# panshengyi/MemVul

Hardware: AMD Instinct MI355X
Metric: issue-reports/sec at seq_len=256 (BERT-base issue encoder + 124-anchor memory match) (higher is better)
Workload: dtype fp16 + fp8 (MV_F16X8: fp16 MFMA sweep + one OCP-e4m3 MFMA correction sweep per GEMM, fp32 accumulate); 1 GPU; BASELINE.json configs[1]: 1xMI355X-per-rank, bert-base-uncased geometry (12 layers), seq_len=256, batch=256, 124-anchor CWE memory, compute dtype MV_F16X8; seeded random-init weights, synthetic token ids resident in HBM; compute=precise, global_batch=256, seq_len=256, anchors=124, parallelism=dp1 (corpus shards, one all-gather of (score,label) stats), stats_transport=none (one rank)

## Files before the change

### memvul_amd/binding.py

```python
from __future__ import annotations

import ctypes as C
import os
import warnings
from typing import Dict, Iterable, Optional, Tuple

import numpy as np

_HERE = os.path.dirname(os.path.abspath(__file__))
LIB_PATH = os.path.join(_HERE, "lib", "libmemvul_hip.so")
LIB_PATH_DEV = os.path.join(_HERE, "lib", "libmemvul_hip_dev.so")
DEV_SWITCHES = ("MEMVUL_GEMM_TILE", "MEMVUL_SHORT_VLO", "MEMVUL_RASTER", "MEMVUL_GN_MAX", "MEMVUL_NUM_CU")

MV_F32, MV_F16, MV_BF16, MV_I32, MV_I64 = 0, 1, 2, 3, 4
MV_F16X8 = 6
COMPUTE_DTYPES = {"f16": MV_F16, "fast": MV_F16, "f16x8": MV_F16X8, "precise": MV_F16X8, "safe": MV_F16X8, "guarded": MV_F16X8,
                  "f32": MV_F32, "reference": MV_F32}
MV_FORM_DEFAULT, MV_FORM_SAFE, MV_FORM_GUARDED = 0, 1, 2
FORMS = {"default": MV_FORM_DEFAULT, "safe": MV_FORM_SAFE, "guarded": MV_FORM_GUARDED}
GUARDED_WARN_SHARE = 0.25
DEFAULT_COMPUTE = "precise"


def default_compute() -> str:
    return os.environ.get("MEMVUL_COMPUTE", DEFAULT_COMPUTE)


def compute_dtype_of(name_or_code) -> int:
    if name_or_code is None:
        name_or_code = default_compute()
    if isinstance(name_or_code, str):
        if name_or_code.lower() not in COMPUTE_DTYPES:
            raise ValueError(f"unknown compute dtype {name_or_code!r}: expected one of {sorted(COMPUTE_DTYPES)}")
        return COMPUTE_DTYPES[name_or_code.lower()]
    if int(name_or_code) not in (MV_F16, MV_F16X8, MV_F32):
        raise ValueError(f"unknown compute dtype code {name_or_code!r}: MV_F16 = {MV_F16}, MV_F16X8 = {MV_F16X8} or MV_F32 = {MV_F32}")
    return int(name_or_code)


def on_sink_policy() -> str:
    v = os.environ.get("MEMVUL_ON_SINK", "warn")
    if v not in ("warn", "safe"):
        raise ValueError(f"MEMVUL_ON_SINK={v!r}: expected 'warn' or 'safe'")
    return v

# ... 607 lines not shown
```

### memvul_amd/csrc/engine.hip

```cpp
#include <hip/hip_runtime.h>
#include <dlfcn.h>
#include <rccl/rccl.h>
#include <unistd.h>

#include <algorithm>
#include <charconv>
#include <chrono>
#include <cmath>
#include <cstdio>
#include <cstdlib>
#include <cstring>
#include <map>
#include <string>
#include <vector>

#include "../../include/memvul_hip.h"
#include "common.h"
#include "gemm.h"
#include "gemm_pp.h"
#include "attention.h"
#include "attention_v2.h"
#include "misc_kernels.h"
#include "match_topk.h"
#include "ref_f32.h"
// ... 158 lines not shown
  int rr = 0;
  Plan plan;
  struct {
    std::vector<int32_t> ids, lens, idx;
    std::vector<float> logits, probs, best, embed;
    std::vector<uint32_t> over;
  } stage, stage2;
  Plan plan2;
  std::vector<uint8_t> last_forms;
  int64_t guard_seqs = 0, guard_rescored = 0;
  float* anchors = nullptr;
  int n_anchors = 0;
  unsigned long long* attn_conc = nullptr;
  unsigned long long* x8_sat = nullptr;

  int32_t *c_ids = nullptr, *c_lens = nullptr;
  std::vector<int32_t> c_lens_host;
  std::vector<void*> pinned;
  int64_t c_n = 0;
  int c_S = 0;
  float* c_best = nullptr;
  int32_t* c_idx = nullptr;
  float* c_psame = nullptr;
  int64_t c_psame_rows = 0;
  int c_G = 0;
  uint32_t* c_over = nullptr;
  std::vector<int16_t> c_pend_w;
  std::vector<uint8_t> c_pend_keep;
  std::vector<uint8_t> c_forms;
  bool c_pending = false;

  bool cls_prune = true;
  int pp_gn_max = 4;
  int pp_raster = 0;
  bool short_vlo = true;
  bool cls_aside = true;
  int cls_min_len = 128;
  int qkv_aside_mask = 0;

  int form = MV_FORM_DEFAULT;

  uint32_t prof_mask = 0xffffffffu;
  bool prof = false;
  std::vector<ProfRec> recs;
  std::vector<hipEvent_t> free_events;

  int gemm_tile = 0;
  int num_cu = 256;

  int dbg_B = 0, dbg_Sp = 0;

  void* rccl_lib = nullptr;
  ncclComm_t comm = nullptr;
  int comm_rank = 0, comm_world = 1;
  decltype(&ncclGetUniqueId) p_ncclGetUniqueId = nullptr;
  decltype(&ncclCommInitRank) p_ncclCommInitRank = nullptr;
  decltype(&ncclAllGather) p_ncclAllGather = nullptr;
  decltype(&ncclCommDestroy) p_ncclCommDestroy = nullptr;
  decltype(&ncclGetErrorString) p_ncclGetErrorString = nullptr;
  decltype(&ncclGetVersion) p_ncclGetVersion = nullptr;
  decltype(&ncclCommCount) p_ncclCommCount = nullptr;
  decltype(&ncclCommUserRank) p_ncclCommUserRank = nullptr;
  void *comm_send = nullptr, *comm_recv = nullptr;
  int64_t comm_send_cap = 0, comm_recv_cap = 0;
};

// ... 87 lines not shown
  hipError_t e = hipGetLastError();
  if (e != hipSuccess) return fail(h, MV_ERR_HIP, std::string("launch ") + what + ": " + hipGetErrorString(e));
  return MV_OK;
}

int choose_gn(int tn, int gn_max) {
  int g = 1;
  for (int d = 1; d <= gn_max && d <= tn; ++d)
    if (tn % d == 0) g = d;
  return g;
}

template <int EPI>
int launch_gemm128(mv_handle* h, hipStream_t stream, int cls, GemmArgs a) {
  if (a.M % 128 || a.N % 128 || a.K % 64) return fail(h, MV_ERR_INVALID, "gemm128: M,N % 128, K % 64 required");
  a.GN = choose_gn(a.N / 128, 8);
  const int grid = (a.M / 128) * (a.N / 128);
  ProfScope ps(h, stream, cls);
  hipLaunchKernelGGL((gemm128_kernel<EPI>), dim3(grid), dim3(256), G128_LDS_BYTES, stream, a);
  return launch_check(h, "gemm128");
}

constexpr int RING64_LDS = 4 * (64 + 64) * 64 * 2;
template <int EPI>
int launch_ring64(mv_handle* h, hipStream_t stream, int cls, GemmArgs a) {
  if (a.M % 64 || a.N % 64 || a.K % 64) return fail(h, MV_ERR_INVALID, "gemm_ring: shape not a multiple of the 64 x 64 x 64 tile");
  a.GN = choose_gn(a.N / 64, 8);
  const int grid = (a.M / 64) * (a.N / 64);
  ProfScope ps(h, stream, cls);
  hipLaunchKernelGGL((gemm_ring_kernel<EPI, 1, 1, 2, 2, 64, 4, 2>), dim3(grid), dim3(256), RING64_LDS, stream, a);
  return launch_check(h, "gemm_ring");
}

template <int PPEPI>
int launch_pp(mv_handle* h, hipStream_t stream, int cls, GemmArgs a) {
  constexpr int RAW = PPEPI != PP_RESLN3;
  if (a.M % 256 || a.N % 256 || a.K % 128 || a.K < 256 || a.N > MV_INTER)
    return fail(h, MV_ERR_INVALID, "gemm_pp: M,N % 256, K % 128, K >= 256, N <= 3072 required");
  if (!a.bias || !a.lnstats) return fail(h, MV_ERR_STATE, "internal: gemm_pp without bias / row statistics");
  if (a.A8 && (a.x8_terms == 1 || a.x8_terms == 3) && a.K % 256)
    return fail(h, MV_ERR_INVALID, "gemm_pp: a weight-side-only fp8 correction sweep needs K % 256 == 0");
  a.GN = choose_gn(a.N / 256, h->pp_gn_max);
  const int tiles = (a.M / 256) * (a.N / 256);
  const int grid = tiles < h->num_cu ? tiles : h->num_cu;
  a.raster_mode = (h->pp_raster == 1 && a.N / 256 > a.GN && ((a.M / 256) * a.GN) % grid == 0) ? 1 : 0;
  const int lds = RAW ? PP_LDS_BYTES_RAW : PP_LDS_BYTES;
  ProfScope ps(h, stream, cls);
  if (a.A8) {
    if (!a.W8 || (PPEPI != PP_QK && !a.out8)) return fail(h, MV_ERR_STATE, "internal: MV_F16X8 GEMM without its fp8 planes");
    hipLaunchKernelGGL((gemm_pp_kernel<PPEPI, RAW, 1>), dim3(grid), dim3(512), lds, stream, a);
  } else {
    hipLaunchKernelGGL((gemm_pp_kernel<PPEPI, RAW, 0>), dim3(grid), dim3(512), lds, stream, a);
  }
  return launch_check(h, "gemm_pp");
}

bool pp_selected(const mv_handle* h, int64_t M) {
  if (M % 256) return false;
  if (h->gemm_tile == 128) return false;
  return h->gemm_tile == 512 || h->precise || (M / 256) * (MV_HIDDEN / 256) >= 256;
}

template <int EPI>
int launch_small(mv_handle* h, hipStream_t stream, int cls, const GemmArgs& a) {
  if (h->gemm_tile == 0 && a.M <= 512 && a.M % 64 == 0 && a.N % 64 == 0) return launch_ring64<EPI>(h, stream, cls, a);
  return launch_gemm128<EPI>(h, stream, cls, a);
}

int pool_head(mv_handle* h, Work& wk, const float* x, size_t row_stride, int B, float* u_out) {
  const unsigned gx = (unsigned)((B + 31) / 32);
  hipLaunchKernelGGL(dense768_kernel<0>, dim3(gx, MV_HIDDEN / 32), dim3(512), 0, wk.stream, x, row_stride, B, h->WpT, h->bp,
                     MV_HIDDEN, h->P == MV_HIDDEN ? u_out : wk.pooled);
  if (int rc = launch_check(h, "pooler")) return rc;
  if (h->P == MV_HIDDEN) return MV_OK;
  hipLaunchKernelGGL(dense768_kernel<1>, dim3(gx, MV_PROJ / 32), dim3(512), 0, wk.stream, wk.pooled, (size_t)MV_HIDDEN, B, h->WhT,
                     h->bh, MV_PROJ, u_out);
  return launch_check(h, "header");
}

// ... 114 lines not shown
  }
  return MV_OK;
}

int encode_dev(mv_handle* h, Work& wk, const int32_t* d_ids, const int32_t* d_lens, int min_len, int B, int S_in, int n_layers, float* u_out,
               const PassForm& pf = PassForm(), bool full = false, int pitch = 0) {
  if (pitch <= 0) pitch = S_in;
  if (h->f32) return encode_f32_dev(h, wk, d_ids, d_lens, B, S_in, n_layers, u_out, pitch);
  const mv_config& c = h->cfg;
  const int Sp = padded_len(S_in);
  const int64_t M = (int64_t)B * Sp, Mpad = round_up(M, 256);
  if (S_in > c.max_pos) return fail(h, MV_ERR_INVALID, "sequence longer than max_pos");
  if (Mpad > h->cap_tokens) return fail(h, MV_ERR_CAPACITY, "B*S exceeds mv_config.max_tokens");
  if (n_layers < 0 || n_layers > c.layers) n_layers = c.layers;
  h->dbg_B = B;
  h->dbg_Sp = Sp;
  const bool big = pp_selected(h, Mpad);
  const bool x8 = h->precise;
  const bool prune = !full && h->cls_prune && u_out && n_layers == c.layers && n_layers > 0;
  const bool one_seq_tiles = Sp == 256 || Sp == 512;
  const bool whole_pass = (Sp == 192 || Sp == 384) && min_len >= h->cls_min_len;
  const bool safe = x8 && pf.safe;
  const bool cls_as = big && x8 && !safe && h->cls_aside && (one_seq_tiles || whole_pass);
  const int qkv_mask = safe ? 7 : h->qkv_aside_mask;
  const bool two_plane = two_plane_pass(h, x8, safe, Sp);
  if (cls_as && one_seq_tiles) {
    const int ntile = (int)(Mpad / 256);
    hipLaunchKernelGGL(cls_tile_flags_kernel, dim3((unsigned)((ntile + 255) / 256)), dim3(256), 0, wk.stream, d_lens, B, Sp, h->cls_min_len, ntile,
                       wk.tile_both);
    if (int rc = launch_check(h, "cls_tile_flags")) return rc;
  }
  const bool special = big && x8;
  auto row_term = [&](const half_t* A, const half_t* W, int N, int K) -> int {
    ProfScope ps(h, wk.stream, KC_CLS_ROW_TERM);
    GemmArgs t{};
    t.M = (int)round_up(2 * B, 64); t.Mreal = 2 * B; t.S = 64; t.A = A; t.W = W; t.N = N; t.K = K; t.outf = wk.cls_corr;
    t.GN = choose_gn(N / 64, 8);
    hipLaunchKernelGGL((gemm_ring_kernel<EPI_F32, 1, 1, 2, 2, 64, 4, 2>), dim3((unsigned)((t.M / 64) * (N / 64))), dim3(256), RING64_LDS, wk.stream, t);
    return launch_check(h, "row term gemm_ring");
  };
  const unsigned ln_grid = (unsigned)((M + 3) / 4);
  {
    ProfScope ps(h, wk.stream, KC_EMBED_LN);
    if (big)
      hipLaunchKernelGGL(embed_ln_kernel<true>, dim3(ln_grid), dim3(256), 0, wk.stream, d_ids, pitch, S_in, Sp, (int)M, c.vocab_size,
                         h->wemb, h->pemb, h->temb, h->embg, h->embb, c.ln_eps, wk.xres, wk.x16, wk.lnstats,
                         x8 ? (half_t*)nullptr : wk.xlo, x8 ? wk.x8 : (uint8_t*)nullptr, h->x8_sat, special ? d_lens : (const int32_t*)nullptr,
                         special ? wk.st_lo : (half_t*)nullptr);
    else
      hipLaunchKernelGGL(embed_ln_kernel<false>, dim3(ln_grid), dim3(256), 0, wk.stream, d_ids, pitch, S_in, Sp, (int)M, c.vocab_size,
                         h->wemb, h->pemb, h->temb, h->embg, h->embb, c.ln_eps, wk.xres, wk.x16, (float*)nullptr,
                         (half_t*)nullptr, (uint8_t*)nullptr, (unsigned long long*)nullptr);
    if (int rc = launch_check(h, "embed_ln")) return rc;
  }
  const float *pend_g = h->embg, *pend_b = h->embb;
  auto run_ln = [&](float* x32, half_t* x16, int rows, const float* g, const float* b) -> int {
    ProfScope ps(h, wk.stream, KC_LN);
    hipLaunchKernelGGL(ln_kernel<true>, dim3((unsigned)((rows + 3) / 4)), dim3(256), 0, wk.stream, x32, x16, rows, g, b, c.ln_eps,
                       (float*)nullptr);
    return launch_check(h, "layernorm");
  };
  auto final_ln = [&](const float* g, const float* b) -> int {
    const size_t n4 = (size_t)M * MV_HIDDEN / 4;
    hipLaunchKernelGGL(hilo_to_f32_kernel, dim3((unsigned)((n4 + 255) / 256)), dim3(256), 0, wk.stream, wk.x16, wk.xlo, n4, wk.xres,
                       special ? (const half_t*)wk.st_lo : (const half_t*)nullptr, Sp, (const uint8_t*)wk.x8);
    if (int rc = launch_check(h, "hilo_to_f32")) return rc;
    return run_ln(wk.xres, wk.x16, (int)M, g, b);
  };
  if (big && n_layers == 0) { if (int rc = final_ln(h->embg, h->embb)) return rc; }
// ... 615 lines not shown
      g_create_error = std::string(name) + "=\"" + e + "\": expected an integer in " + std::to_string(lo) + " .. " + std::to_string(hi);
      return false;
    }
    *out = (int)v;
    return true;
  };
  auto env_flag = [&](const char* name, bool* out) -> bool {
    int v = *out ? 1 : 0;
    if (!env_int(name, 0, 1, &v)) return false;
    *out = v != 0;
    return true;
  };
  {
    int ns = h->n_streams;
    if (!env_int("MEMVUL_STREAMS", 1, 2, &ns)) return MV_ERR_INVALID;
    h->n_streams = h->n_alloc = ns;
  }
  for (int wi = 0; wi < h->n_alloc; ++wi) {
    e = hipStreamCreateWithFlags(&h->work[wi].stream, hipStreamNonBlocking);
    if (e != hipSuccess) {
      g_create_error = std::string("hipStreamCreate: ") + hipGetErrorString(e);
      return MV_ERR_HIP;
    }
  }
  hipFuncSetAttribute((const void*)gemm_ring_kernel<EPI_F32, 1, 1, 2, 2, 64, 4, 2>, hipFuncAttributeMaxDynamicSharedMemorySize, RING64_LDS);
  hipFuncSetAttribute((const void*)gemm_ring_kernel<EPI_QKV, 1, 1, 2, 2, 64, 4, 2>, hipFuncAttributeMaxDynamicSharedMemorySize, RING64_LDS);
  hipFuncSetAttribute((const void*)gemm_ring_kernel<EPI_GELU, 1, 1, 2, 2, 64, 4, 2>, hipFuncAttributeMaxDynamicSharedMemorySize, RING64_LDS);
  hipFuncSetAttribute((const void*)gemm_ring_kernel<EPI_RES, 1, 1, 2, 2, 64, 4, 2>, hipFuncAttributeMaxDynamicSharedMemorySize, RING64_LDS);
  hipFuncSetAttribute((const void*)gemm_pp_kernel<PP_QK, 1, 0>, hipFuncAttributeMaxDynamicSharedMemorySize, PP_LDS_BYTES_RAW);
  hipFuncSetAttribute((const void*)gemm_pp_kernel<PP_GELU, 1, 0>, hipFuncAttributeMaxDynamicSharedMemorySize, PP_LDS_BYTES_RAW);
  hipFuncSetAttribute((const void*)gemm_pp_kernel<PP_RESLN3, 0, 0>, hipFuncAttributeMaxDynamicSharedMemorySize, PP_LDS_BYTES);
  hipFuncSetAttribute((const void*)gemm_pp_kernel<PP_QK, 1, 1>, hipFuncAttributeMaxDynamicSharedMemorySize, PP_LDS_BYTES_RAW);
  hipFuncSetAttribute((const void*)gemm_pp_kernel<PP_GELU, 1, 1>, hipFuncAttributeMaxDynamicSharedMemorySize, PP_LDS_BYTES_RAW);
  hipFuncSetAttribute((const void*)gemm_pp_kernel<PP_RESLN3, 0, 1>, hipFuncAttributeMaxDynamicSharedMemorySize, PP_LDS_BYTES);
#define MV_ATT_ATTR(NKB, NCH)                                                                                                     \
  hipFuncSetAttribute((const void*)attention_v2_kernel<NKB, NCH, 0>, hipFuncAttributeMaxDynamicSharedMemorySize, ATT2_LDS_BYTES(NKB)); \
  hipFuncSetAttribute((const void*)attention_v2_kernel<NKB, NCH, 1>, hipFuncAttributeMaxDynamicSharedMemorySize, ATT2_LDS_BYTES(NKB))
  MV_ATT_ATTR(1, 1); MV_ATT_ATTR(2, 1); MV_ATT_ATTR(3, 1); MV_ATT_ATTR(4, 1); MV_ATT_ATTR(2, 3); MV_ATT_ATTR(2, 4);
#undef MV_ATT_ATTR
  hipFuncSetAttribute((const void*)attention_v2_kernel<1, 1, 1, 1>, hipFuncAttributeMaxDynamicSharedMemorySize, ATT2_LDS_BYTES_VLO(1));
  hipFuncSetAttribute((const void*)attention_v2_kernel<2, 1, 1, 1>, hipFuncAttributeMaxDynamicSharedMemorySize, ATT2_LDS_BYTES_VLO(2));
  hipFuncSetAttribute((const void*)attention_v2_kernel<1, 3, 1, 1>, hipFuncAttributeMaxDynamicSharedMemorySize, ATT2_LDS_BYTES_VLO(1));
  hipFuncSetAttribute((const void*)attention_v2_kernel<2, 2, 1, 1>, hipFuncAttributeMaxDynamicSharedMemorySize, ATT2_LDS_BYTES_VLO(2));
  hipFuncSetAttribute((const void*)attention_v2_kernel<2, 3, 1, 1>, hipFuncAttributeMaxDynamicSharedMemorySize, ATT2_LDS_BYTES_VLO(2));
  hipFuncSetAttribute((const void*)attention_v2_kernel<2, 4, 1, 1>, hipFuncAttributeMaxDynamicSharedMemorySize, ATT2_LDS_BYTES_VLO(2));
  (void)hipGetLastError();
  if (!env_flag("MEMVUL_CLS_PRUNE", &h->cls_prune)) return MV_ERR_INVALID;
  if (const char* e = getenv("MEMVUL_QKV_ASIDE")) {
    h->qkv_aside_mask = 0;
    if (strcmp(e, "none")) {
      for (const char* c = e; *c; ++c) {
        const int bit = (*c == 'q' || *c == 'Q') ? 1 : (*c == 'k' || *c == 'K') ? 2 : (*c == 'v' || *c == 'V') ? 4 : 0;
        if (!bit) {
          g_create_error = std::string("MEMVUL_QKV_ASIDE=\"") + e + "\": expected a subset of \"qkv\", \"\" or \"none\"";
          return MV_ERR_INVALID;
        }
        h->qkv_aside_mask |= bit;
      }
    }
  }
  if (!env_flag("MEMVUL_CLS_ASIDE", &h->cls_aside)) return MV_ERR_INVALID;
  if (!env_int("MEMVUL_CLS_ASIDE_MIN_LEN", 1, 512, &h->cls_min_len)) return MV_ERR_INVALID;
  if (const char* e = getenv("MEMVUL_FORM")) {
    if (!strcmp(e, "safe")) h->form = MV_FORM_SAFE;
    else if (!strcmp(e, "default")) h->form = MV_FORM_DEFAULT;
    else if (!strcmp(e, "guarded")) h->form = MV_FORM_GUARDED;
    else {
      g_create_error = std::string("MEMVUL_FORM=\"") + e + "\": expected \"default\", \"safe\" or \"guarded\"";
      return MV_ERR_INVALID;
    }
  }
  {
    int ncu = 0;
    if (hipDeviceGetAttribute(&ncu, hipDeviceAttributeMultiprocessorCount, device) == hipSuccess && ncu > 0) h->num_cu = ncu;
  }
#ifdef MEMVUL_DEV_SWITCHES
  {
    int gt = h->gemm_tile;
    if (!env_int("MEMVUL_GEMM_TILE", 0, 512, &gt)) return MV_ERR_INVALID;
    if (gt != 0 && gt != 128 && gt != 512) { g_create_error = "MEMVUL_GEMM_TILE: expected 0, 128 or 512"; return MV_ERR_INVALID; }
    h->gemm_tile = gt;
    if (!env_flag("MEMVUL_SHORT_VLO", &h->short_vlo)) return MV_ERR_INVALID;
    if (!env_int("MEMVUL_GN_MAX", 1, 12, &h->pp_gn_max)) return MV_ERR_INVALID;
    if (!env_int("MEMVUL_RASTER", 0, 1, &h->pp_raster)) return MV_ERR_INVALID;
    if (!env_int("MEMVUL_NUM_CU", 1, h->num_cu, &h->num_cu)) return MV_ERR_INVALID;
  }
#endif

  h->cap_tokens = round_up(cfg->max_tokens, 256) + 256;
  const int64_t T = h->cap_tokens;
  int rc = MV_OK;
  auto A = [&](int r) { if (rc == MV_OK) rc = r; };
  const int64_t BG = (int64_t)cfg->max_batch * cfg->max_anchors;
  const int64_t Bp = round_up(cfg->max_batch, 256);
  for (int wi = 0; wi < h->n_alloc; ++wi) {
    Work& wk = h->work[wi];
    A(dev_alloc(h, wk.stream, &wk.d_ids, T));
    A(dev_alloc(h, wk.stream, &wk.d_lens, (int64_t)cfg->max_batch + 16));
    A(dev_alloc(h, wk.stream, &wk.seq_over, (int64_t)cfg->max_batch));
    A(dev_alloc(h, wk.stream, &wk.d_idx, (int64_t)cfg->max_batch));
    A(dev_alloc(h, wk.stream, &wk.xres, T * MV_HIDDEN));
    A(dev_alloc(h, wk.stream, &wk.x16, T * MV_HIDDEN));
    A(dev_alloc(h, wk.stream, &wk.q, T * MV_HIDDEN));
    A(dev_alloc(h, wk.stream, &wk.k, T * MV_HIDDEN));
    A(dev_alloc(h, wk.stream, &wk.vt, T * MV_HIDDEN));
    A(dev_alloc(h, wk.stream, &wk.ctx, T * MV_HIDDEN));
    A(dev_alloc(h, wk.stream, &wk.h16, T * MV_INTER));
    A(dev_alloc(h, wk.stream, &wk.lnstats, T * 6));
    A(dev_alloc(h, wk.stream, &wk.lnpart, T * 6));
    A(dev_alloc(h, wk.stream, &wk.c32, Bp * MV_HIDDEN));
    A(dev_alloc(h, wk.stream, &wk.cq, Bp * MV_HIDDEN));
    A(dev_alloc(h, wk.stream, &wk.c16, Bp * MV_HIDDEN));
    A(dev_alloc(h, wk.stream, &wk.cctx, Bp * MV_HIDDEN));
    A(dev_alloc(h, wk.stream, &wk.ch16, Bp * MV_INTER));
    A(dev_alloc(h, wk.stream, &wk.u, (int64_t)cfg->max_batch * h->P));
    A(dev_alloc(h, wk.stream, &wk.pooled, (int64_t)cfg->max_batch * MV_HIDDEN));
    A(dev_alloc(h, wk.stream, &wk.u_in, (int64_t)cfg->max_batch * h->P));
// ... 781 lines not shown

int mv_debug_read(mv_handle* h, int buffer, void* dst, int64_t bytes) try {
  if (!h || !dst || bytes <= 0) return MV_ERR_INVALID;
  Work& wk = h->work[0];
  const int64_t T = (int64_t)h->dbg_B * h->dbg_Sp;
  const void* src = nullptr;
  int64_t avail = 0;
  if (h->f32 && buffer >= 1 && buffer <= 9)
    return fail(h, MV_ERR_INVALID, "mv_debug_read: buffers 1 - 9 are the fp16 planes of MV_F16 / MV_F16X8; an MV_F32 handle has buffer 0 (hidden fp32) and 10 (embedding)");
  switch (buffer) {
    case 0: src = wk.xres; avail = T * MV_HIDDEN * 4; break;
    case 1: src = wk.x16; avail = T * MV_HIDDEN * 2; break;
    case 2: src = wk.q; avail = T * MV_HIDDEN * 2; break;
    case 3: src = wk.k; avail = T * MV_HIDDEN * 2; break;
    case 4: src = wk.vt; avail = T * MV_HIDDEN * 2; break;
    case 5: src = wk.ctx; avail = T * MV_HIDDEN * 2; break;
    case 6: src = wk.h16; avail = T * MV_INTER * 2; break;
    case 7: src = wk.q_lo; avail = T * MV_HIDDEN * 2; break;
    case 8: src = wk.k_lo; avail = T * MV_HIDDEN * 2; break;
    case 9: src = wk.vt_lo; avail = T * MV_HIDDEN * 2; break;
    case 10: src = wk.u; avail = (int64_t)h->dbg_B * h->P * 4; break;
    default: return fail(h, MV_ERR_INVALID, "mv_debug_read: unknown buffer");
  }
  if (!src) return fail(h, MV_ERR_STATE, "mv_debug_read: this buffer does not exist in this compute dtype");
  if (bytes > avail) return fail(h, MV_ERR_INVALID, "mv_debug_read: more bytes requested than the buffer holds");
  HIPCHK(h, hipMemcpyAsync(dst, src, (size_t)bytes, hipMemcpyDeviceToHost, wk.stream));
  HIPCHK(h, hipStreamSynchronize(wk.stream));
  return MV_OK;
} catch (...) { return on_exception(h); }

int mv_test_gemm(mv_handle* h, int variant, int M, int N, int K, const uint16_t* A, const uint16_t* W, const float* bias,
                 float* C, int iters, float* ms) try {
  if (!h || !A || !W || M <= 0 || N <= 0 || K <= 0) return fail(h, MV_ERR_INVALID, "mv_test_gemm: bad argument");
  if (variant != 0 && variant != 19) return fail(h, MV_ERR_INVALID, "mv_test_gemm: variant 0 (128^2 tile) or 19 (64^2 ring)");
  if (variant == 0 && (M % 128 || N % 128 || K % 64)) return fail(h, MV_ERR_INVALID, "mv_test_gemm: M,N % 128 and K % 64 required");
  HIPCHK(h, hipSetDevice(h->device));
  const hipStream_t s0 = h->work[0].stream;
  half_t *dA = nullptr, *dW = nullptr;
  float *dB = nullptr, *dC = nullptr;
  int rc;
  if ((rc = dev_alloc(h, s0, &dA, (int64_t)M * K, false))) return rc;
  if ((rc = dev_alloc(h, s0, &dW, (int64_t)N * K, false))) return rc;
  if ((rc = dev_alloc(h, s0, &dB, N))) return rc;
  if ((rc = dev_alloc(h, s0, &dC, (int64_t)M * N))) return rc;
  HIPCHK(h, hipMemcpyAsync(dA, A, (size_t)M * K * 2, hipMemcpyHostToDevice, s0));
  HIPCHK(h, hipMemcpyAsync(dW, W, (size_t)N * K * 2, hipMemcpyHostToDevice, s0));
  if (bias) HIPCHK(h, hipMemcpyAsync(dB, bias, (size_t)N * 4, hipMemcpyHostToDevice, s0));
  GemmArgs g{};
  g.A = dA; g.W = dW; g.bias = dB; g.M = M; g.Mreal = M; g.N = N; g.K = K; g.outf = dC; g.S = 64;
  if (iters < 1) iters = 1;
  hipEvent_t e0, e1;
  hipEventCreate(&e0);
  hipEventCreate(&e1);
  auto run = [&]() -> int { return variant == 0 ? launch_gemm128<EPI_F32>(h, s0, KC_TEST_GEMM, g) : launch_ring64<EPI_F32>(h, s0, KC_TEST_GEMM, g); };
  rc = run();
  if (rc == MV_OK) {
    hipEventRecord(e0, s0);
    for (int i = 0; i < iters && rc == MV_OK; ++i) rc = run();
    hipEventRecord(e1, s0);
  }
  hipError_t se = hipStreamSynchronize(s0);
  float t = 0.f;
  hipEventElapsedTime(&t, e0, e1);
  hipEventDestroy(e0);
  hipEventDestroy(e1);
  if (ms) *ms = t / (float)iters;
  if (rc == MV_OK && se != hipSuccess) rc = fail(h, MV_ERR_HIP, std::string("test gemm: ") + hipGetErrorString(se));
  if (rc == MV_OK && C) {
    se = hipMemcpy(C, dC, (size_t)M * N * 4, hipMemcpyDeviceToHost);
    if (se != hipSuccess) rc = fail(h, MV_ERR_HIP, std::string("test gemm copy: ") + hipGetErrorString(se));
  }
  dev_free(h, dA); dev_free(h, dW); dev_free(h, dB); dev_free(h, dC);
  return rc;
} catch (...) { return on_exception(h); }

int mv_test_gemm_f32(mv_handle* h, int act, int M, int N, int K, const float* A, const float* W, const float* bias, const float* res, float* C, int iters,
                     float* ms) try {
  if (!h || !A || !W || M <= 0 || N <= 0 || K <= 0) return fail(h, MV_ERR_INVALID, "mv_test_gemm_f32: bad argument");
  if (act < RF_ACT_NONE || act > RF_ACT_RES || (act == RF_ACT_RES && !res)) return fail(h, MV_ERR_INVALID, "mv_test_gemm_f32: act 0 (bias), 1 (GELU) or 2 (+ res, res required)");
  if (M % 128 || N % 128 || K % 32) return fail(h, MV_ERR_INVALID, "mv_test_gemm_f32: M,N % 128 and K % 32 required");
  HIPCHK(h, hipSetDevice(h->device));
  const hipStream_t s0 = h->work[0].stream;
  float *dA = nullptr, *dW = nullptr, *dB = nullptr, *dR = nullptr, *dC = nullptr;
  int rc;
  if ((rc = dev_alloc(h, s0, &dA, (int64_t)M * K, false))) return rc;
  if ((rc = dev_alloc(h, s0, &dW, (int64_t)N * K, false))) return rc;
  if ((rc = dev_alloc(h, s0, &dB, N))) return rc;
// ... 202 lines not shown
```

### memvul_amd/csrc/gemm.h

```cpp
#pragma once
#include "common.h"

enum { EPI_F32 = 0, EPI_QKV = 1, EPI_GELU = 2, EPI_RES = 3 };

struct GemmArgs {
  const half_t* A;
  const half_t* W;
  const float* bias;
  int M;
  int Mreal;
  int N, K;
  int GN;
  float* outf;
  half_t* out16;
  half_t* out16b;
  float* xres;
  half_t* q;
  half_t* k;
  half_t* vt;
  int S;
  int col0;
  const float* lnstats;
  const float* lng;
  const float* lnb;
  float* lnpart;
  float ln_eps;
  const uint8_t* A8;
  const uint8_t* W8;
  uint8_t* out8;
  int x8_scale;
  int x8_terms;
  int x8_aside_mask;
  half_t* vt_lo;
  half_t *q_lo, *k_lo;
  unsigned long long* x8_sat;
  int raster_mode;
  int out8_hi_only;
  const int* tile_both;
  const float* cls_corr;
  half_t* sp_lo_out;
  half_t* vlo_sp;
};

__device__ __forceinline__ void raster(int t, int tm_count, int tn_count, int GN, int& tile_m, int& tile_n) {
  const int per_group = tm_count * GN;
  const int g = t / per_group;
  const int r = t - g * per_group;
  tile_m = r / GN;
  tile_n = g * GN + (r - tile_m * GN);
}

template <int EPI>
__device__ __forceinline__ void epilogue_frag(const GemmArgs& a, const floatx16& acc, int mb, int nb, int lane) {
  const int hi = lane >> 5;
  const int n = nb + (lane & 31);
  if constexpr (EPI == EPI_F32) {
#pragma unroll
    for (int r = 0; r < 16; ++r) a.outf[(size_t)(mb + mfma32_row(r, hi)) * a.N + n] = acc[r];
  } else if constexpr (EPI == EPI_GELU) {
#pragma unroll
    for (int r = 0; r < 16; ++r) a.out16[(size_t)(mb + mfma32_row(r, hi)) * a.N + n] = (half_t)gelu_erf(acc[r]);
  } else if constexpr (EPI == EPI_RES) {
    const int lane_off = 4 * hi * MV_HIDDEN + (lane & 31);
#pragma unroll
    for (int r = 0; r < 16; ++r) {
      float* rowbase = a.xres + (size_t)(mb + (r & 3) + 8 * (r >> 2)) * MV_HIDDEN + nb;
      rowbase[lane_off] = acc[r];
    }
  } else {
    const int which = (nb + a.col0) / MV_HIDDEN;
    const int hn = nb + a.col0 - which * MV_HIDDEN;
    const int head = hn >> 6;
// ... 202 lines not shown
#pragma unroll
        for (int j = 0; j < FR_N; ++j)
          acc[i][j] = __builtin_amdgcn_mfma_f32_32x32x16_f16(fa[i], fb[j], acc[i][j], 0, 0, 0);
    }
  };

  const int nk = K / BK;
#pragma unroll
  for (int s = 0; s < STAGES - 1; ++s)
    if (s < nk) stage(s, s);
  int slot = 0, fill = STAGES - 1;
  for (int kt = 0; kt < nk; ++kt) {
    const int newer = nk - 1 - kt;
    if (STAGES >= 5 && newer >= 3) wait_vmcnt<(STAGES >= 5 ? 3 : 0) * G>();
    else if (STAGES >= 4 && newer >= 2) wait_vmcnt<(STAGES >= 4 ? 2 : 0) * G>();
    else if (STAGES >= 3 && newer >= 1) wait_vmcnt<(STAGES >= 3 ? 1 : 0) * G>();
    else wait_vmcnt<0>();
    asm volatile("s_waitcnt lgkmcnt(0)" ::: "memory");
    __builtin_amdgcn_s_barrier();
    asm volatile("" ::: "memory");
    if (kt + STAGES - 1 < nk) stage(fill, kt + STAGES - 1);
    compute(slot);
    asm volatile("" ::: "memory");
    slot = (slot + 1 == STAGES) ? 0 : slot + 1;
    fill = (fill + 1 == STAGES) ? 0 : fill + 1;
  }

#pragma unroll
  for (int i = 0; i < FR_M; ++i)
#pragma unroll
    for (int j = 0; j < FR_N; ++j)
      epilogue_frag<EPI>(a, acc[i][j], m0 + (wm * FR_M + i) * 32, n0 + (wn * FR_N + j) * 32, lane);
}
```

### memvul_amd/csrc/gemm_pp.h

```cpp
#pragma once
#include "common.h"
#include <type_traits>
#include "gemm.h"

enum { PP_QK = 1, PP_GELU = 3, PP_RESLN3 = 8 };
constexpr int PP_F = 4;

#define PP_LDS_A 0
#define PP_LDS_B 65536
#define PP_LDS_BIAS 131072
#define PP_LDS_SCR (PP_LDS_BIAS + MV_INTER * 4)
#define PP_LDS_BYTES (PP_LDS_SCR + 8 * 2048)
#define PP_LDS_BIAS_T PP_LDS_BIAS
#define PP_LDS_STATS (PP_LDS_BIAS + 2048)
#define PP_LDS_SCR_RAW (PP_LDS_STATS + 2 * 6144)
#define PP_LDS_RSTD (PP_LDS_SCR_RAW + 8 * 2048)
#define PP_LDS_BYTES_RAW (PP_LDS_RSTD + 2048)

__device__ __forceinline__ uint32_t pack_h2(float a, float b) {
  const half2_t h = {(half_t)a, (half_t)b};
  return __builtin_bit_cast(uint32_t, h);
}

__device__ __forceinline__ void pin_f32x4(float& a, float& b, float& c, float& d) {
#if defined(__HIP_DEVICE_COMPILE__)
  asm("" : "+v"(a), "+v"(b), "+v"(c), "+v"(d));
#endif
}

__device__ __forceinline__ uint32_t f2u(float x) { return __float_as_uint(x); }
__device__ __forceinline__ float u2f(uint32_t x) { return __uint_as_float(x); }
typedef uint32_t u32x2 __attribute__((ext_vector_type(2)));
typedef uint32_t u32x4 __attribute__((ext_vector_type(4)));
typedef int intx4 __attribute__((ext_vector_type(4)));
typedef int intx8 __attribute__((ext_vector_type(8)));

__device__ __forceinline__ void scr_f16x2(uint32_t w0, uint32_t w1, uint32_t w2, uint32_t w3, const u32x2 (&da)[4],
                                          const u32x2 (&db)[4], uint32_t r, u32x4 (&o)[4]) {
#if defined(__HIP_DEVICE_COMPILE__)
  asm volatile(
      "ds_write_b64 %4, %8\n\tds_write_b64 %5, %9\n\tds_write_b64 %6, %10\n\tds_write_b64 %7, %11\n\t"
      "ds_read_b128 %0, %16\n\tds_read_b128 %1, %16 offset:1024\n\t"
      "ds_write_b64 %4, %12\n\tds_write_b64 %5, %13\n\tds_write_b64 %6, %14\n\tds_write_b64 %7, %15\n\t"
      "ds_read_b128 %2, %16\n\tds_read_b128 %3, %16 offset:1024\n\ts_waitcnt lgkmcnt(0)"
      : "=&v"(o[0]), "=&v"(o[1]), "=&v"(o[2]), "=&v"(o[3])
// ... 52 lines not shown
}
__device__ __forceinline__ void scr_f16_rev2(uint32_t wc, const u32x4& a0, const u32x4& a1, const u32x4& b0, const u32x4& b1, uint32_t r0,
                                             uint32_t r1, uint32_t r2, uint32_t r3, u32x2 (&oa)[4], u32x2 (&ob)[4]) {
#if defined(__HIP_DEVICE_COMPILE__)
  asm volatile(
      "ds_write_b128 %8, %9\n\tds_write_b128 %8, %10 offset:1024\n\t"
      "ds_read_b64 %0, %13\n\tds_read_b64 %1, %14\n\tds_read_b64 %2, %15\n\tds_read_b64 %3, %16\n\t"
      "ds_write_b128 %8, %11\n\tds_write_b128 %8, %12 offset:1024\n\t"
      "ds_read_b64 %4, %13\n\tds_read_b64 %5, %14\n\tds_read_b64 %6, %15\n\tds_read_b64 %7, %16\n\ts_waitcnt lgkmcnt(0)"
      : "=&v"(oa[0]), "=&v"(oa[1]), "=&v"(oa[2]), "=&v"(oa[3]), "=&v"(ob[0]), "=&v"(ob[1]), "=&v"(ob[2]), "=&v"(ob[3])
      : "v"(wc), "v"(a0), "v"(a1), "v"(b0), "v"(b1), "v"(r0), "v"(r1), "v"(r2), "v"(r3)
      : "memory");
  __builtin_amdgcn_sched_barrier(0);
#endif
}


__device__ __forceinline__ void lds_read_bgb1(uint32_t addr, float4& bi, float4& ga, float4& be) {
#if defined(__HIP_DEVICE_COMPILE__)
  asm volatile("ds_read_b128 %0, %3\n\tds_read_b128 %1, %3 offset:3072\n\tds_read_b128 %2, %3 offset:6144\n\ts_waitcnt lgkmcnt(0)"
               : "=&v"(bi), "=&v"(ga), "=&v"(be)
               : "v"(addr)
               : "memory");
  __builtin_amdgcn_sched_barrier(0);
#endif
}

__device__ __forceinline__ int sload_i32(const int* p) {
  int v = 0;
#if defined(__HIP_DEVICE_COMPILE__)
  asm volatile("s_load_dword %0, %1, 0x0\n\ts_waitcnt lgkmcnt(0)" : "=s"(v) : "s"(p) : "memory");
#endif
  return v;
}

__device__ __forceinline__ void raster_pp(const GemmArgs& a, int L, int G, int tm_count, int tn_count, int& tile_m, int& tile_n) {
  if (a.raster_mode == 1) {
    const int ngroups = tn_count / a.GN;
    const int w = L / G, r = L - w * G;
    const int b = w / ngroups, g = w - b * ngroups;
    const int p = b * G + r;
    tile_m = p / a.GN;
    tile_n = g * a.GN + (p - tile_m * a.GN);
  } else {
    raster(L, tm_count, tn_count, a.GN, tile_m, tile_n);
  }
}

template <int EPI, int RAW = 0, int X8 = 0>
__global__ __launch_bounds__(512, 2) void gemm_pp_kernel(GemmArgs a) {
  static_assert(EPI == PP_QK || EPI == PP_GELU || EPI == PP_RESLN3, "kernel kinds of the encoder layer");
  static_assert(RAW == (EPI != PP_RESLN3), "PP_QK / PP_GELU consume the raw stream (virtual LayerNorm), PP_RESLN3 produces it");
  constexpr bool IS_RES = (EPI == PP_RESLN3);
  static_assert(X8 == 0 || X8 == 1, "X8 = 1: MV_F16X8 (the fp8 correction sweep)");
  constexpr int WAITN = 2 * PP_F;
  constexpr int LDS_SCR = RAW ? PP_LDS_SCR_RAW : PP_LDS_SCR;
  extern __shared__ __attribute__((aligned(16))) char smem[];
  const int tid = threadIdx.x;
  const int lane = tid & 63;
  const int hi = lane >> 5, l31 = lane & 31;
  const int wave = __builtin_amdgcn_readfirstlane(tid >> 6);
  const int wr = wave >> 2, wc = wave & 3;
  const int K = a.K, nk0 = K >> 6;
  constexpr int nseg = X8 ? 2 : 1;
  auto short_tile = [&](int tm) -> bool { return a.tile_both && sload_i32(a.tile_both + tm) != 0; };
  auto both_terms = [&](int tm, int tn) -> bool {
// ... 236 lines not shown
    if constexpr (X8) {
#if defined(__HIP_DEVICE_COMPILE__)
      constexpr int P = s & 3, a0 = (P >= 2) ? 4 : 0, bq = (P == 1 || P == 2) ? 2 : 0;
      asm volatile("" : "+v"(acc[a0][bq]), "+v"(acc[a0 + 1][bq]), "+v"(acc[a0 + 2][bq]), "+v"(acc[a0 + 3][bq]), "+v"(acc[a0][bq + 1]),
                   "+v"(acc[a0 + 1][bq + 1]), "+v"(acc[a0 + 2][bq + 1]), "+v"(acc[a0 + 3][bq + 1]));
#endif
    }
    asm volatile("s_waitcnt vmcnt(%0)" ::"n"(WAITN) : "memory");
    __builtin_amdgcn_sched_barrier(0);
    __builtin_amdgcn_s_barrier();
    __builtin_amdgcn_sched_barrier(0);
  };

  auto issue_stats = [&](int itn, int tm, int tn) {
    if (itn * G + bslot < ntiles && wave < 4) {
#pragma unroll
      for (int pc = 0; pc < 2; ++pc) {
        const int piece = 2 * wave + pc;
        if (piece < 6) {
          const char* src = (const char*)a.lnstats + (size_t)tm * 6144 + piece * 1024 + lane * 16;
          glds16((const half_t*)src, smem + PP_LDS_STATS + (itn & 1) * 6144 + piece * 1024);
        } else if (piece == 6) {
          const char* src = (const char*)a.bias + (size_t)tn * 1024 + lane * 16;
          glds16((const half_t*)src, smem + PP_LDS_BIAS_T + (itn & 1) * 1024);
        }
      }
    }
  };
  if constexpr (RAW) {
    int tm = 0, tn = 0;
    if (bslot < ntiles) raster_pp(a, bslot, G, tm_count, tn_count, tm, tn);
    issue_stats(0, tm, tn);
  }

  issue_psi(std::integral_constant<int, 0>{});
  issue_psi(std::integral_constant<int, 1>{});
  issue_psi(std::integral_constant<int, 2>{});
  issue_psi(std::integral_constant<int, 3>{});
  issue_psi(std::integral_constant<int, 4>{});
  issue_psi(std::integral_constant<int, 5>{});
  issue_psi(std::integral_constant<int, 6>{});
  asm volatile("s_waitcnt vmcnt(%0) lgkmcnt(0)" ::"n"(WAITN) : "memory");
  __builtin_amdgcn_sched_barrier(0);
  __builtin_amdgcn_s_barrier();
  __builtin_amdgcn_sched_barrier(0);

  auto run_tiles = [&](auto grpc) {
  for (int it = 0;; ++it) {
    const int L = it * G + bslot;
    if (L >= ntiles) break;
    int tile_m, tile_n;
    raster_pp(a, L, G, tm_count, tn_count, tile_m, tile_n);
    int next_m = 0, next_n = 0;
    const bool has_next = L + G < ntiles;
    if (has_next) raster_pp(a, L + G, G, tm_count, tn_count, next_m, next_n);
    const int mw = (tile_m << 8) + wr * 128;
    const int nw = (tile_n << 8) + wc * 64;
    bool tile_short = false;
    if constexpr (X8) tile_short = short_tile(tile_m);
    const bool tile_both_terms = X8 && (a.x8_terms == 1 ? tile_short : both_terms(tile_m, tile_n));

    {
      const uint32_t baddr = (uint32_t)(PP_LDS_BIAS + (nw + 4 * q4) * 4);
      const uint32_t scr = (uint32_t)(LDS_SCR + wave * 2048);
      const uint32_t sf = (uint32_t)((m16 >> 2) & 3);
      const uint32_t scr_c = scr + (lane >> 2) * 64 + ((((uint32_t)lane & 3) ^ (((uint32_t)lane >> 4) & 3)) << 4);
// ... 79 lines not shown
          }
      }
    }

    if constexpr (decltype(grpc)::value == 0) read_set(std::integral_constant<int, 0>{});
    auto two_ktiles = [&](auto f8c, bool last) {
      interval(std::integral_constant<int, 0>{}, grpc, f8c);
      interval(std::integral_constant<int, 1>{}, grpc, f8c);
      interval(std::integral_constant<int, 2>{}, grpc, f8c);
      interval(std::integral_constant<int, 3>{}, grpc, f8c);
      interval(std::integral_constant<int, 4>{}, grpc, f8c);
      interval(std::integral_constant<int, 5>{}, grpc, f8c);
      interval(std::integral_constant<int, 6>{}, grpc, f8c);
      interval(std::integral_constant<int, 7>{}, grpc, f8c, last);
    };
    for (int kt = 0; kt < nk0; kt += 2) {
      if constexpr (RAW) {
        if (kt == 2) {
          issue_stats(it + 1, next_m, next_n);
          if (wave >= 4) {
            const int row = (wave - 4) * 64 + lane;
            const uint32_t saddr = (uint32_t)(PP_LDS_STATS + (it & 1) * 6144 + row * 24);
            float2 p0, p1, p2;
            asm volatile("ds_read_b64 %0, %3\n\tds_read_b64 %1, %3 offset:8\n\tds_read_b64 %2, %3 offset:16\n\ts_waitcnt lgkmcnt(0)"
                         : "=&v"(p0), "=&v"(p1), "=&v"(p2)
                         : "v"(saddr)
                         : "memory");
            const float rs = ln_from_partials(p0, p1, p2, a.ln_eps).y;
            const uint32_t waddr = (uint32_t)(PP_LDS_RSTD + (it & 1) * 1024 + row * 4);
            asm volatile("ds_write_b32 %0, %1" ::"v"(waddr), "v"(rs) : "memory");
          }
        }
      }
      two_ktiles(std::false_type{}, !X8 && kt + 2 >= nk0);
    }
    if constexpr (X8) {
      const int nk = nk0 + (tile_both_terms ? nk0 : nk0 >> 1);
      for (int kt = nk0; kt < nk; kt += 2) two_ktiles(std::true_type{}, kt + 2 >= nk);
    }

    {
      const uint32_t scr = (uint32_t)(LDS_SCR + wave * 2048);
      const uint32_t sf = (uint32_t)((m16 >> 2) & 3);
      const uint32_t scr_c = scr + (lane >> 2) * 64 + ((((uint32_t)lane & 3) ^ (((uint32_t)lane >> 4) & 3)) << 4);
      const int crow = lane >> 2, cchunk = lane & 3;
      int cls_b[2] = {-1, -1};
      if constexpr (X8) {
        if (a.cls_corr || a.sp_lo_out || a.vlo_sp) {
#pragma unroll
          for (int j = 0; j < 2; ++j) {
            const int row = mw + 64 * j, b = row / a.S;
            if (row < a.Mreal && b * a.S == row) cls_b[j] = b;
          }
        }
        if (a.cls_corr && !tile_both_terms) {
#pragma unroll
          for (int j = 0; j < 2; ++j) {
            if (cls_b[j] >= 0 && m16 < 2) {
              const float* cp = a.cls_corr + (size_t)(2 * cls_b[j] + m16) * a.N + nw + 4 * q4;
              floatx4 c[4];
#pragma unroll
              for (int cb = 0; cb < 4; ++cb) c[cb] = *(const floatx4*)(cp + 16 * cb);
#if defined(__HIP_DEVICE_COMPILE__)
              asm volatile("" : "+v"(c[0]), "+v"(c[1]), "+v"(c[2]), "+v"(c[3]));
#endif
#pragma unroll
              for (int cb = 0; cb < 4; ++cb) {
                acc[4 * j][cb][0] = __builtin_fmaf(c[cb][0], 1.0f / 2048.0f, acc[4 * j][cb][0]);
                acc[4 * j][cb][1] = __builtin_fmaf(c[cb][1], 1.0f / 2048.0f, acc[4 * j][cb][1]);
                acc[4 * j][cb][2] = __builtin_fmaf(c[cb][2], 1.0f / 2048.0f, acc[4 * j][cb][2]);
                acc[4 * j][cb][3] = __builtin_fmaf(c[cb][3], 1.0f / 2048.0f, acc[4 * j][cb][3]);
              }
            }
          }
        }
      }
      if constexpr (IS_RES) {
#pragma unroll
        for (int tb = 0; tb < 8; ++tb) {
          float s1 = 0.f, s2 = 0.f;
#pragma unroll
          for (int cb = 0; cb < 4; ++cb)
#pragma unroll
            for (int e = 0; e < 4; ++e) {
              const float v = acc[tb][cb][e];
              s1 += v;
              s2 = __builtin_fmaf(v, v, s2);
            }
// ... 265 lines not shown
```

Before: 14500 issue-reports/s.

## Add dedicated row-term MFMA kernel and stage CLS correction via LDS prefetch

Replaces the 64x64 ring GEMM used for the small CLS row-term correction with a dedicated register-pipelined 32x32 MFMA kernel that streams A and W fragments directly from global memory without LDS. In the fp8-corrected pp GEMM, the per-tile CLS correction rows are prefetched into LDS mid-K-loop by two waves and read back in the epilogue, instead of each wave loading them from global memory at the end. Both paths are on by default (form 3) and aim to cut the row-term launch cost and the epilogue global-load latency. The trade-off is a larger LDS footprint for the RESLN3 variant and extra inline asm that must index correctly.

```diff
diff --git a/memvul_amd/binding.py b/memvul_amd/binding.py
--- a/memvul_amd/binding.py
+++ b/memvul_amd/binding.py
@@ -10,7 +10,7 @@
 _HERE = os.path.dirname(os.path.abspath(__file__))
 LIB_PATH = os.path.join(_HERE, "lib", "libmemvul_hip.so")
 LIB_PATH_DEV = os.path.join(_HERE, "lib", "libmemvul_hip_dev.so")
-DEV_SWITCHES = ("MEMVUL_GEMM_TILE", "MEMVUL_SHORT_VLO", "MEMVUL_RASTER", "MEMVUL_GN_MAX", "MEMVUL_NUM_CU")
+DEV_SWITCHES = ("MEMVUL_GEMM_TILE", "MEMVUL_SHORT_VLO", "MEMVUL_RASTER", "MEMVUL_GN_MAX", "MEMVUL_NUM_CU", "MEMVUL_ROW_TERM")
 
 MV_F32, MV_F16, MV_BF16, MV_I32, MV_I64 = 0, 1, 2, 3, 4
 MV_F16X8 = 6
diff --git a/memvul_amd/csrc/engine.hip b/memvul_amd/csrc/engine.hip
--- a/memvul_amd/csrc/engine.hip
+++ b/memvul_amd/csrc/engine.hip
@@ -214,6 +214,7 @@
 
   bool cls_prune = true;
   int pp_gn_max = 4;
+  int row_term_form = 3;
   int pp_raster = 0;
   bool short_vlo = true;
   bool cls_aside = true;
@@ -367,6 +368,16 @@
   return launch_check(h, "gemm_ring");
 }
 
+template <int WM, int WN, int D>
+int launch_row_term_t(mv_handle* h, hipStream_t stream, int cls, const GemmArgs& a) {
+  if (a.Mreal <= 0 || a.N % (32 * WN) || a.K % 64) return fail(h, MV_ERR_INVALID, "row_term: N % 32 WN, K % 64 required");
+  const int grid = ((a.Mreal + 32 * WM - 1) / (32 * WM)) * (a.N / (32 * WN));
+  ProfScope ps(h, stream, cls);
+  hipLaunchKernelGGL((row_term_kernel<WM, WN, D>), dim3((unsigned)grid), dim3(64 * WM * WN), 0, stream, a);
+  return launch_check(h, "row_term");
+}
+int launch_row_term(mv_handle* h, hipStream_t stream, int cls, const GemmArgs& a) { return launch_row_term_t<1, 2, 6>(h, stream, cls, a); }
+
 template <int PPEPI>
 int launch_pp(mv_handle* h, hipStream_t stream, int cls, GemmArgs a) {
   constexpr int RAW = PPEPI != PP_RESLN3;
@@ -379,7 +390,8 @@
   const int tiles = (a.M / 256) * (a.N / 256);
   const int grid = tiles < h->num_cu ? tiles : h->num_cu;
   a.raster_mode = (h->pp_raster == 1 && a.N / 256 > a.GN && ((a.M / 256) * a.GN) % grid == 0) ? 1 : 0;
-  const int lds = RAW ? PP_LDS_BYTES_RAW : PP_LDS_BYTES;
+  a.cls_lds = (h->row_term_form & 2) && a.A8 && a.cls_corr && a.S % 256 == 0 && a.K >= 384;
+  const int lds = RAW ? PP_LDS_BYTES_RAW : (a.A8 ? PP_LDS_BYTES_CORR : PP_LDS_BYTES);
   ProfScope ps(h, stream, cls);
   if (a.A8) {
     if (!a.W8 || (PPEPI != PP_QK && !a.out8)) return fail(h, MV_ERR_STATE, "internal: MV_F16X8 GEMM without its fp8 planes");
@@ -560,9 +572,10 @@
   }
   const bool special = big && x8;
   auto row_term = [&](const half_t* A, const half_t* W, int N, int K) -> int {
-    ProfScope ps(h, wk.stream, KC_CLS_ROW_TERM);
     GemmArgs t{};
     t.M = (int)round_up(2 * B, 64); t.Mreal = 2 * B; t.S = 64; t.A = A; t.W = W; t.N = N; t.K = K; t.outf = wk.cls_corr;
+    if (h->row_term_form & 1) return launch_row_term(h, wk.stream, KC_CLS_ROW_TERM, t);
+    ProfScope ps(h, wk.stream, KC_CLS_ROW_TERM);
     t.GN = choose_gn(N / 64, 8);
     hipLaunchKernelGGL((gemm_ring_kernel<EPI_F32, 1, 1, 2, 2, 64, 4, 2>), dim3((unsigned)((t.M / 64) * (N / 64))), dim3(256), RING64_LDS, wk.stream, t);
     return launch_check(h, "row term gemm_ring");
@@ -1244,7 +1257,7 @@
   hipFuncSetAttribute((const void*)gemm_pp_kernel<PP_RESLN3, 0, 0>, hipFuncAttributeMaxDynamicSharedMemorySize, PP_LDS_BYTES);
   hipFuncSetAttribute((const void*)gemm_pp_kernel<PP_QK, 1, 1>, hipFuncAttributeMaxDynamicSharedMemorySize, PP_LDS_BYTES_RAW);
   hipFuncSetAttribute((const void*)gemm_pp_kernel<PP_GELU, 1, 1>, hipFuncAttributeMaxDynamicSharedMemorySize, PP_LDS_BYTES_RAW);
-  hipFuncSetAttribute((const void*)gemm_pp_kernel<PP_RESLN3, 0, 1>, hipFuncAttributeMaxDynamicSharedMemorySize, PP_LDS_BYTES);
+  hipFuncSetAttribute((const void*)gemm_pp_kernel<PP_RESLN3, 0, 1>, hipFuncAttributeMaxDynamicSharedMemorySize, PP_LDS_BYTES_CORR);
 #define MV_ATT_ATTR(NKB, NCH)                                                                                                     \
   hipFuncSetAttribute((const void*)attention_v2_kernel<NKB, NCH, 0>, hipFuncAttributeMaxDynamicSharedMemorySize, ATT2_LDS_BYTES(NKB)); \
   hipFuncSetAttribute((const void*)attention_v2_kernel<NKB, NCH, 1>, hipFuncAttributeMaxDynamicSharedMemorySize, ATT2_LDS_BYTES(NKB))
@@ -1295,6 +1308,7 @@
     if (!env_flag("MEMVUL_SHORT_VLO", &h->short_vlo)) return MV_ERR_INVALID;
     if (!env_int("MEMVUL_GN_MAX", 1, 12, &h->pp_gn_max)) return MV_ERR_INVALID;
     if (!env_int("MEMVUL_RASTER", 0, 1, &h->pp_raster)) return MV_ERR_INVALID;
+    if (!env_int("MEMVUL_ROW_TERM", 0, 3, &h->row_term_form)) return MV_ERR_INVALID;
     if (!env_int("MEMVUL_NUM_CU", 1, h->num_cu, &h->num_cu)) return MV_ERR_INVALID;
   }
 #endif
@@ -2142,7 +2156,7 @@
 int mv_test_gemm(mv_handle* h, int variant, int M, int N, int K, const uint16_t* A, const uint16_t* W, const float* bias,
                  float* C, int iters, float* ms) try {
   if (!h || !A || !W || M <= 0 || N <= 0 || K <= 0) return fail(h, MV_ERR_INVALID, "mv_test_gemm: bad argument");
-  if (variant != 0 && variant != 19) return fail(h, MV_ERR_INVALID, "mv_test_gemm: variant 0 (128^2 tile) or 19 (64^2 ring)");
+  if (variant != 0 && variant != 19 && variant != 20) return fail(h, MV_ERR_INVALID, "mv_test_gemm: variant 0 (128^2 tile), 19 (64^2 ring) or 20 (row term)");
   if (variant == 0 && (M % 128 || N % 128 || K % 64)) return fail(h, MV_ERR_INVALID, "mv_test_gemm: M,N % 128 and K % 64 required");
   HIPCHK(h, hipSetDevice(h->device));
   const hipStream_t s0 = h->work[0].stream;
@@ -2162,7 +2176,13 @@
   hipEvent_t e0, e1;
   hipEventCreate(&e0);
   hipEventCreate(&e1);
-  auto run = [&]() -> int { return variant == 0 ? launch_gemm128<EPI_F32>(h, s0, KC_TEST_GEMM, g) : launch_ring64<EPI_F32>(h, s0, KC_TEST_GEMM, g); };
+  auto run = [&]() -> int {
+    switch (variant) {
+      case 0: return launch_gemm128<EPI_F32>(h, s0, KC_TEST_GEMM, g);
+      case 19: return launch_ring64<EPI_F32>(h, s0, KC_TEST_GEMM, g);
+      default: return launch_row_term(h, s0, KC_TEST_GEMM, g);
+    }
+  };
   rc = run();
   if (rc == MV_OK) {
     hipEventRecord(e0, s0);
diff --git a/memvul_amd/csrc/gemm.h b/memvul_amd/csrc/gemm.h
--- a/memvul_amd/csrc/gemm.h
+++ b/memvul_amd/csrc/gemm.h
@@ -38,6 +38,7 @@
   int out8_hi_only;
   const int* tile_both;
   const float* cls_corr;
+  int cls_lds;
   half_t* sp_lo_out;
   half_t* vlo_sp;
 };
@@ -306,3 +307,79 @@
     for (int j = 0; j < FR_N; ++j)
       epilogue_frag<EPI>(a, acc[i][j], m0 + (wm * FR_M + i) * 32, n0 + (wn * FR_N + j) * 32, lane);
 }
+
+template <int WM, int WN, int D>
+__global__ __launch_bounds__(64 * WM * WN, 2) void row_term_kernel(GemmArgs a) {
+  const int lane = threadIdx.x & 63;
+  const int wave = __builtin_amdgcn_readfirstlane(threadIdx.x >> 6);
+  const int hi = lane >> 5;
+  const int tm_count = (a.Mreal + 32 * WM - 1) / (32 * WM);
+  const int t = xcd_remap(blockIdx.x, gridDim.x);
+  const int tile_n = t / tm_count, tile_m = t - tile_n * tm_count;
+  const int wm = wave / WN, wn = wave - wm * WN;
+  const int mb = (tile_m * WM + wm) * 32, nb = (tile_n * WN + wn) * 32;
+  if (mb >= a.Mreal) return;
+  const int K = a.K;
+  const int arow = min(mb + (lane & 31), a.Mreal - 1);
+  const half_t* pa = a.A + (size_t)arow * K + 8 * hi;
+  const half_t* pw = a.W + (size_t)(nb + (lane & 31)) * K + 8 * hi;
+  floatx16 acc;
+  init_frag<EPI_F32>(a, acc, mb, nb, lane);
+
+  half8_t fa[D][4], fb[D][4];
+  auto load = [&](int s, int g) {
+#pragma unroll
+    for (int kk = 0; kk < 4; ++kk) {
+      fa[s][kk] = *(const half8_t*)(pa + g * 64 + kk * 16);
+      fb[s][kk] = *(const half8_t*)(pw + g * 64 + kk * 16);
+    }
+  };
+  auto compute = [&](int s) {
+#pragma unroll
+    for (int kk = 0; kk < 4; ++kk) acc = __builtin_amdgcn_mfma_f32_32x32x16_f16(fa[s][kk], fb[s][kk], acc, 0, 0, 0);
+  };
+  const int nk = K >> 6;
+  if (nk % D == 0) {
+#pragma unroll
+    for (int s = 0; s < D; ++s) load(s, s);
+    for (int g0 = D; g0 < nk; g0 += D) {
+#pragma unroll
+      for (int s = 0; s < D; ++s) {
+        __builtin_amdgcn_sched_barrier(0);
+        compute(s);
+        __builtin_amdgcn_sched_barrier(0);
+        load(s, g0 + s);
+        __builtin_amdgcn_sched_barrier(0);
+      }
+    }
+#pragma unroll
+    for (int s = 0; s < D; ++s) {
+      __builtin_amdgcn_sched_barrier(0);
+      compute(s);
+    }
+  } else {
+#pragma unroll
+    for (int s = 0; s < D; ++s)
+      if (s < nk) load(s, s);
+    for (int g0 = 0; g0 < nk; g0 += D) {
+#pragma unroll
+      for (int s = 0; s < D; ++s) {
+        const int g = g0 + s;
+        if (g < nk) {
+          __builtin_amdgcn_sched_barrier(0);
+          compute(s);
+          __builtin_amdgcn_sched_barrier(0);
+          if (g + D < nk) load(s, g + D);
+          __builtin_amdgcn_sched_barrier(0);
+        }
+      }
+    }
+  }
+
+  const int n = nb + (lane & 31);
+#pragma unroll
+  for (int r = 0; r < 16; ++r) {
+    const int row = mb + mfma32_row(r, hi);
+    if (row < a.Mreal) a.outf[(size_t)row * a.N + n] = acc[r];
+  }
+}
diff --git a/memvul_amd/csrc/gemm_pp.h b/memvul_amd/csrc/gemm_pp.h
--- a/memvul_amd/csrc/gemm_pp.h
+++ b/memvul_amd/csrc/gemm_pp.h
@@ -11,6 +11,8 @@
 #define PP_LDS_BIAS 131072
 #define PP_LDS_SCR (PP_LDS_BIAS + MV_INTER * 4)
 #define PP_LDS_BYTES (PP_LDS_SCR + 8 * 2048)
+#define PP_LDS_CORR PP_LDS_BYTES
+#define PP_LDS_BYTES_CORR (PP_LDS_CORR + 2048)
 #define PP_LDS_BIAS_T PP_LDS_BIAS
 #define PP_LDS_STATS (PP_LDS_BIAS + 2048)
 #define PP_LDS_SCR_RAW (PP_LDS_STATS + 2 * 6144)
@@ -129,6 +131,20 @@
   asm volatile("s_load_dword %0, %1, 0x0\n\ts_waitcnt lgkmcnt(0)" : "=s"(v) : "s"(p) : "memory");
 #endif
   return v;
+}
+
+__device__ __forceinline__ void lds_read_corr(uint32_t sbase, floatx4 (&c)[4]) {
+#if defined(__HIP_DEVICE_COMPILE__)
+  uint32_t t0, t1;
+  asm volatile(
+      "v_mbcnt_lo_u32_b32 %4, -1, 0\n\tv_mbcnt_hi_u32_b32 %4, -1, %4\n\t"
+      "v_and_b32 %5, 1, %4\n\tv_lshlrev_b32 %5, 10, %5\n\tv_and_or_b32 %4, %4, 48, %5\n\tv_add_u32 %4, %6, %4\n\t"
+      "ds_read_b128 %0, %4\n\tds_read_b128 %1, %4 offset:64\n\tds_read_b128 %2, %4 offset:128\n\tds_read_b128 %3, %4 offset:192\n\t"
+      "s_waitcnt lgkmcnt(0)"
+      : "=&v"(c[0]), "=&v"(c[1]), "=&v"(c[2]), "=&v"(c[3]), "=&v"(t0), "=&v"(t1)
+      : "s"(sbase)
+      : "memory");
+#endif
 }
 
 __device__ __forceinline__ void raster_pp(const GemmArgs& a, int L, int G, int tm_count, int tn_count, int& tile_m, int& tile_n) {
@@ -431,6 +447,14 @@
     if (bslot < ntiles) raster_pp(a, bslot, G, tm_count, tn_count, tm, tn);
     issue_stats(0, tm, tn);
   }
+  const bool cls_lds = X8 && a.cls_corr && a.cls_lds;
+  auto issue_corr = [&](int it, int tm, int tn) {
+    if (wave == 4 || wave == 5) {
+      const int b = min((tm << 8) / a.S, (a.Mreal - 1) / a.S);
+      const char* src = (const char*)(a.cls_corr + (size_t)(2 * b + (wave - 4)) * a.N + (tn << 8)) + lane * 16;
+      glds16((const half_t*)src, smem + (RAW ? PP_LDS_STATS + (it & 1) * 6144 : PP_LDS_CORR) + (wave - 4) * 1024);
+    }
+  };
 
   issue_psi(std::integral_constant<int, 0>{});
   issue_psi(std::integral_constant<int, 1>{});
@@ -576,6 +600,9 @@
           }
         }
       }
+      if constexpr (X8) {
+        if (kt == 4 && cls_lds) issue_corr(it, tile_m, tile_n);
+      }
       two_ktiles(std::false_type{}, !X8 && kt + 2 >= nk0);
     }
     if constexpr (X8) {
@@ -597,7 +624,16 @@
             if (row < a.Mreal && b * a.S == row) cls_b[j] = b;
           }
         }
-        if (a.cls_corr && !tile_both_terms) {
+        if (cls_lds) {
+          if (!tile_both_terms && cls_b[0] >= 0) {
+            floatx4 c[4];
+            lds_read_corr((uint32_t)((RAW ? PP_LDS_STATS + (it & 1) * 6144 : PP_LDS_CORR) + wc * 256), c);
+#pragma unroll
+            for (int cb = 0; cb < 4; ++cb)
+#pragma unroll
+              for (int e = 0; e < 4; ++e) acc[0][cb][e] = m16 < 2 ? __builtin_fmaf(c[cb][e], 1.0f / 2048.0f, acc[0][cb][e]) : acc[0][cb][e];
+          }
+        } else if (a.cls_corr && !tile_both_terms) {
 #pragma unroll
           for (int j = 0; j < 2; ++j) {
             if (cls_b[j] >= 0 && m16 < 2) {
```

After: 14210 issue-reports/s. -2.0%, worse.
